# pku-lab-1806-llm/lab-1806-vec-db

Measured on AMD Instinct MI355X. Metric: queries/sec at recall@10, Gist1M d=960 (Flat brute force, L2Sqr, k=10), higher is better.
Workload: dtype f32 (int8 lower-bound filter pass); 1 GPU; flat_knn_gist1m; rows=1000000, dim=960, k=10, dist=L2Sqr, parallelism=single GPU, steps_in_flight=1, queries_per_corpus_pass=128

## Files before the change

lab_1806_vec_db_amd/csrc/api.hip:

```cpp
#include <algorithm>
#include <cmath>
#include <cstring>

#include "ctx.hpp"
#include "pq_hnsw.hpp"

using namespace vdb;

static thread_local std::string g_last_error;
void vdb::set_last_error(const std::string &m) { g_last_error = m; }
void vdb::require_gpu() {
    int cnt = 0;
    hipError_t e = hipGetDeviceCount(&cnt);
    if (e != hipSuccess || cnt <= 0)
        throw Error(VDB_ERR_NOGPU, std::string("no usable HIP device (libvdbhip has no CPU fallback): ") +
                                       hipGetErrorString(e));
}

void vdb::merge_topk_dev(Index &ix, const void *d_dists, const void *d_ids, const void *d_counts, uint64_t stride_d,
                           uint64_t stride_i, uint64_t stride_c, uint64_t n_shards, uint64_t nq, uint64_t k,
                           void *d_out_idx, void *d_out_dist, void *d_out_count, void *stream) {
    VDB_REQUIRE(d_dists && d_ids && d_counts && d_out_idx && d_out_dist && d_out_count, "null argument");
    VDB_REQUIRE(k >= 1 && k <= 1024, "k must be in 1..1024");
    VDB_REQUIRE(nq <= 65535 && n_shards <= 65535, "too many queries or shards for one call");
// ... 414 lines not shown
    idx->ix.flat_mode = mode;
    VDB_API_END
}
int vdb_set_param(vdb_index *idx, const char *name, int64_t value) {
    VDB_API_BEGIN
    VDB_REQUIRE(idx && name, "null argument");
    std::string n(name);
    if (n == "mfma_variant")
        mfma_set_variant((int)value);
    else if (n == "flat_share")
        mfma_set_share((int)value);
    else if (n == "flat_gemm")
        idx->ix.flat_gemm_mode = (int)value;
    else if (n == "hnsw_dma")
        hnsw_set_dma((int)value);
    else if (n == "hnsw_half")
        hnsw_set_half((int)value);
    else if (n == "ivf_half")
        ivf_set_half((int)value);
    else if (n == "ivf_q8")
        ivf_set_q8((int)value);
    else if (n == "hnsw_build_gpu")
        hnsw_set_build_gpu((int)value);
    else if (n == "hnsw_pool_cap")
        hnsw_set_pool_cap((int)value);
    else if (n == "pq_adc_fast")
        pq_set_adc_fast((int)value);
    else if (n == "pq_sample16")
        pq_set_adc16_sample((int)value);
    else if (n == "pq_adc16")
        pq_set_adc16((int)value);
    else if (n == "pq_adc8_sliced")
        pq_set_adc8_sliced((int)value);
    else if (n == "flat_sample_thin")
        mfma_set_sample_thin((int)value);
    else if (n == "flat_gemm_tw")
        gemm_set_tw((int)value);
    else if (n == "flat_gemm_nt")
        gemm_set_nt((int)value);
    else if (n == "flat_gemm_zigzag")
        gemm_set_zigzag((int)value);
    else if (n == "flat_gemm_block_rows") {
        VDB_REQUIRE(value >= 0, "flat_gemm_block_rows must be >= 0");
        gemm_set_block_rows((uint64_t)value);
    }
    else if (n == "flat_gemm_stagger")
        gemm_set_stagger((int)value);
    else if (n == "flat_gemm_debug")
        idx->ix.flat_gemm_debug = (int)value;
    else if (n == "flat_tail")
        idx->ix.flat_tail_mode = (int)value;
    else if (n == "flat_tail_lb_nw")
        flat_tail_lb_set_nw((int)value);
    else if (n == "flat_small")
        idx->ix.flat_small_mode = (int)value;
    else if (n == "flat_small_max_rows")
        idx->ix.flat_small_max_rows = (uint64_t)value;
    else if (n == "flat_half")
        idx->ix.flat_half_mode = (int)value;
    else if (n == "flat_i8")
        idx->ix.flat_i8_mode = (int)value;
    else if (n == "flat_i8_rows") {
        VDB_REQUIRE(value >= 64 && value <= 8192 && value % 64 == 0, "flat_i8_rows must be a multiple of 64 in [64, 8192]");
        idx->ix.flat_i8_kprime = (uint32_t)value;
    }
    else if (n == "debug_alloc_fail_over")
        devbuf_fail_over() = (size_t)value;
    else if (n == "flat_i8_unit_min")
        idx->ix.flat_i8_unit_min = (int)value;
    else if (n == "flat_i8_full")
        idx->ix.flat_i8_full = (int)value;
    else if (n == "flat_i8_refine") {
        idx->ix.flat_i8_refine = (int)value;
        idx->ix.i8_refine_on = 0;
        idx->ix.i8_refine_calls = 0;
    }
    else if (n == "flat_i8_second")
        idx->ix.flat_i8_second = (int)value;
    else if (n == "flat_i8_stats") {
        idx->ix.flat_i8_stats = (int)value;
        for (auto &h : idx->ix.i8_rounds_hist) h = 0;
        idx->ix.i8_hits_sum = 0;
        idx->ix.i8_hits_max = 0;
        idx->ix.i8_stat_queries = 0;
    }
    else if (n == "flat_i8_hits") {
        VDB_REQUIRE(value >= 256 && value <= 4096, "flat_i8_hits must be in [256, 4096]");
        idx->ix.flat_i8_hits = (uint32_t)value;
    }
    else if (n == "flat_gemm8_sample_res")
        gemm8_set_sample_res((int)value);
    else if (n == "flat_gemm8_nt")
        gemm8_set_nt((int)value);
    else if (n == "flat_gemm8_kc")
        gemm8_set_kc((int)value);
    else if (n == "flat_gemm8_burst")
        gemm8_set_burst((int)value);
    else if (n == "flat_gemm8_res")
        gemm8_set_res((int)value);
    else if (n == "flat_gemm8_coop")
        gemm8_set_coop((int)value);
    else if (n == "flat_gemm8_grid")
        gemm8_set_grid((int)value);
    else if (n == "flat_gemm_coop")
        gemm_set_coop((int)value);
    else if (n == "flat_half_kmul") {
        VDB_REQUIRE(value >= 1 && value <= 64, "flat_half_kmul must be in [1, 64]");
        idx->ix.flat_half_kmul = (uint32_t)value;
    }
    else
        throw Error(VDB_ERR_INVALID, "unknown parameter " + n);
    VDB_API_END
}
int vdb_index_prepare(vdb_index *idx, int all_tiers) {
    VDB_API_BEGIN
    VDB_REQUIRE(idx, "null index");
    require_gpu();
    idx->ix.prepare_flat(all_tiers != 0);
    VDB_API_END
}
int vdb_flat_fallback_count(const vdb_index *idx, uint64_t *out) {
    VDB_API_BEGIN
    VDB_REQUIRE(idx && out, "null argument");
    *out = idx->ix.fallback_count.load();
    VDB_API_END
}

int vdb_get_stat(const vdb_index *idx, const char *name, uint64_t *out) {
    VDB_API_BEGIN
    VDB_REQUIRE(idx && name && out, "null argument");
    std::string n(name);
    if (n == "flat_fallback")
        *out = idx->ix.fallback_count.load();
    else if (n == "flat_half_queries")
        *out = idx->ix.half_queries.load();
    else if (n == "flat_half_redo")
        *out = idx->ix.half_redo.load();
    else if (n == "flat_half_valid")
        *out = idx->ix.half_valid ? 1 : 0;
    else if (n == "flat_gemm_coop_sets")
        *out = gemm_last_coop();
    else if (n == "flat_gemm8_coop_sets")
        *out = gemm8_last_coop();
    else if (n == "flat_i8_queries")
        *out = idx->ix.i8_queries.load();
    else if (n == "flat_i8_redo")
        *out = idx->ix.i8_redo.load();
    else if (n == "flat_i8_valid")
        *out = idx->ix.i8_valid.load() ? 1 : 0;
    else if (n.rfind("flat_i8_rounds_", 0) == 0 && n.size() == 16 && n[15] >= '0' && n[15] <= '8')
        *out = idx->ix.i8_rounds_hist[n[15] - '0'].load();
    else if (n == "mirror_alloc_failures")
        *out = idx->ix.mirror_alloc_failures.load();
    else if (n == "flat_i8_second_queries")
        *out = idx->ix.i8_second_queries.load();
    else if (n == "flat_i8_second_redo")
        *out = idx->ix.i8_second_redo.load();
    else if (n == "flat_i8_hits_sum")
        *out = idx->ix.i8_hits_sum.load();
    else if (n == "flat_i8_hits_max")
        *out = idx->ix.i8_hits_max.load();
    else if (n == "flat_i8_stat_queries")
        *out = idx->ix.i8_stat_queries.load();
    else if (n == "flat_i8_rows_walked")
        *out = idx->ix.i8_rows_walked.load();
    else if (n == "flat_bf16_mirror")
        *out = idx->ix.tiled_built ? 1 : 0;
    else if (n == "hnsw_heap_walk_queries")
        *out = idx->ix.hnsw.heap_walk_queries.load();
    else if (n == "hnsw_half_dropped")
        *out = idx->ix.hnsw.last_half_dropped.load();
    else if (n == "ivf_last_offers")
        *out = idx->ix.ivf.last_offers.load();
    else if (n == "ivf_last_rows_fetched_q8")
        *out = idx->ix.ivf.last_rows_fetched_q8.load();
    else if (n == "ivf_last_kept_q8")
        *out = idx->ix.ivf.last_kept_q8.load();
    else if (n == "ivf_last_kept")
        *out = idx->ix.ivf.last_kept.load();
    else if (n == "pq_adc16_queries")
        *out = idx->ix.pq.adc16_queries.load();
    else if (n == "flat_i8_refine_queries")
        *out = idx->ix.i8_refine_queries.load();
    else if (n == "flat_i8_refine_on")
        *out = (uint64_t)idx->ix.i8_refine_on.load();
    else if (n == "pq_q8_overflow")
        *out = idx->ix.pq.q8_overflow.load();
    else if (n == "pq_q8_short")
        *out = idx->ix.pq.q8_short.load();
    else if (n == "pq_q8_hits_sum")
        *out = idx->ix.pq.q8_hits_sum.load();
    else if (n == "pq_q8_hits_max")
        *out = idx->ix.pq.q8_hits_max.load();
    else if (n == "hbm_bytes_per_row")
        *out = idx->ix.hbm_bytes_per_row();
    else
        throw Error(VDB_ERR_INVALID, "unknown statistic " + n);
    VDB_API_END
}

int vdb_pq_attach(vdb_index *idx, uint64_t n_bits, uint64_t m, const float *centroids, const uint8_t *codes) {
    VDB_API_BEGIN
    VDB_REQUIRE(idx && centroids, "null argument");
    pq_attach(idx->ix, n_bits, m, centroids, codes);
    VDB_API_END
}
int vdb_pq_build(vdb_index *idx, uint64_t n_bits, uint64_t m, uint64_t train_n, uint64_t max_iter, float tol,
                 uint64_t seed) {
    VDB_API_BEGIN
    VDB_REQUIRE(idx, "null index");
    pq_build(idx->ix, n_bits, m, train_n, max_iter, tol, seed);
    VDB_API_END
}
int vdb_pq_clear(vdb_index *idx) {
    VDB_API_BEGIN
    VDB_REQUIRE(idx, "null index");
    pq_clear(idx->ix);
    VDB_API_END
}
int vdb_pq_has(const vdb_index *idx, int *out) {
    VDB_API_BEGIN
    VDB_REQUIRE(idx && out, "null argument");
    *out = idx->ix.pq.present ? 1 : 0;
    VDB_API_END
}
int vdb_pq_info(const vdb_index *idx, uint64_t *n_bits, uint64_t *m, uint64_t *enc_dim) {
    VDB_API_BEGIN
    VDB_REQUIRE(idx, "null index");
    VDB_REQUIRE(idx->ix.pq.present, "no PQ table");
    if (n_bits) *n_bits = idx->ix.pq.n_bits;
    if (m) *m = idx->ix.pq.m;
    if (enc_dim) *enc_dim = idx->ix.pq.enc_dim;
    VDB_API_END
}
int vdb_pq_export(const vdb_index *idx, float *centroids, uint8_t *codes) {
    VDB_API_BEGIN
    VDB_REQUIRE(idx, "null index");
    const Index &ix = idx->ix;
    VDB_REQUIRE(ix.pq.present, "no PQ table");
    if (centroids) std::memcpy(centroids, ix.pq.h_centroids.data(), ix.pq.h_centroids.size() * sizeof(float));
    if (codes && ix.n) {
        ix.use_device();
        VDB_HIP(hipMemcpy(codes, ix.pq.d_codes.p, ix.n * ix.pq.enc_dim, hipMemcpyDeviceToHost));
    }
// ... 460 lines not shown
```

lab_1806_vec_db_amd/csrc/index.hip:

```cpp
#include "index.hpp"

#include <algorithm>
#include <cmath>
#include <cstring>

namespace vdb {

Index::Index(int dev, uint64_t d, int ds, bool u8) : device(dev), dim(d), dist(ds), elem_u8(u8) {
#ifndef VDB_HOST_SANITIZER_BUILD
    use_device();
    hipDeviceProp_t prop;
    VDB_HIP(hipGetDeviceProperties(&prop, dev));
    num_cu = prop.multiProcessorCount > 0 ? prop.multiProcessorCount : 256;
    std::string arch = prop.gcnArchName;
    if (arch.rfind("gfx950", 0) != 0)
        throw Error(4, "libvdbhip is built for gfx950 (MI355X) only; device reports " + arch);
#endif
}

std::unique_ptr<Workspace> Index::acquire_ws() {
    use_device();
    {
        std::lock_guard<std::mutex> g(ws_mu);
        if (!ws_free.empty()) {
// ... 626 lines not shown
                                     ws.dense.as<float>(), ld_s, num_cu, s, unit_min ? 1 : 0);
        else if (gemm)
            launch_flat_gemm_sample(xt, n, (uint32_t)dim, ws.qfrag_g.as<float>(), d_qmul, (uint32_t)ngroups,
                                    d_sq.as<float>(), cosine, s_step, ws.dense.as<float>(), ld_s, num_cu, s);
        else
            launch_flat_mfma_sample(d_tiled.as<float>(), n, (uint32_t)dim, ws.qfrag.as<float>(), (uint32_t)nbatch,
                                    d_sq.as<float>(), cosine, s_step, ws.dense.as<float>(), ld_s, num_cu, s);
        if (n_s <= select_tau_max_n()) {
            launch_select_tau(ws.dense.as<float>(), ld_s, (uint32_t)n_s, (uint32_t)nq_pad, (uint32_t)nq, s_rank, d_tau, s);
        } else {
            const uint32_t cap_s = topk_capacity(s_rank);
            launch_topk_dense(ws.dense.as<float>(), ld_s, n_s, (uint32_t)nq_pad, s_rank, ws.lists.as<uint64_t>(), s);
            launch_topk_merge(ws.lists.as<uint64_t>(), nl_s, cap_s, (uint32_t)nq_pad, s_rank, ws.keys_a.as<uint64_t>(), s);
            launch_extract_tau(ws.keys_a.as<uint64_t>(), cap_s, (uint32_t)nq_pad, s_rank, d_tau, s);
        }
        if (nq_pad > nq && n_s > select_tau_max_n())
            VDB_HIP(hipMemsetD32Async(reinterpret_cast<hipDeviceptr_t>(d_tau + nq), (int)0xFF800000u, nq_pad - nq, s));
    }
    uint64_t *d_cand = ws.lists.as<uint64_t>();
    uint32_t *d_sync = d_hits + nq_pad;
    if (!half && !i8) VDB_HIP(hipMemsetAsync(d_hits, 0, (nq_pad + sync_words) * sizeof(uint32_t), s));
    const uint64_t hbm_passes = gemm ? ngroups : (nbatch + mfma_share() - 1) / mfma_share();
    {
        std::lock_guard<std::mutex> g(pass_mu);
        if (pass_ev_valid) VDB_HIP(hipStreamWaitEvent(s, pass_ev, 0));
    }
    prof_begin(ws, i8 ? "flat_i8" : (half ? "flat_half" : "flat_mfma"),
               double(hbm_passes) * double(n) * dim * (i8 ? 1 : (half ? sizeof(uint16_t) : sizeof(float))));
    if (i8)
        launch_flat_gemm8_filter(d_tiled_i8.p, n, (uint32_t)dim, ws.qfrag_g.p, d_qscale, (uint32_t)ngroups, d_rowc_i8.as<float>(), d_tau,
                                 d_cand, d_hits, CAND_CAP, flat_gemm_debug, num_cu, s,
                                 i8_second ? CAND_CAP : std::max<uint32_t>(64u, s_step * s_rank));
    else if (gemm)
        launch_flat_gemm_filter(xt, n, (uint32_t)dim, ws.qfrag_g.as<float>(), d_qmul, (uint32_t)ngroups,
                                d_sq.as<float>(), cosine, d_tau, d_cand, d_hits, CAND_CAP, flat_gemm_debug, num_cu, s);
    else
        launch_flat_mfma_filter(d_tiled.as<float>(), n, (uint32_t)dim, ws.qfrag.as<float>(), (uint32_t)nbatch,
                                d_sq.as<float>(), cosine, d_tau, d_cand, d_hits, CAND_CAP, d_sync, num_cu, s);
    prof_end(ws);
    {
        std::lock_guard<std::mutex> g(pass_mu);
        if (!pass_ev) VDB_HIP(hipEventCreateWithFlags(&pass_ev, hipEventDisableTiming));
        VDB_HIP(hipEventRecord(pass_ev, s));
        pass_ev_valid = true;
    }
    SplitErr se;
    if (half) {
        se.qerr = d_qerr;
        se.dx_abs = half_dx_abs;
        se.dx_rel = half_dx_rel;
    }
    if (i8) {
        se.qoff = d_qoff;
        se.mu_norm = i8_mu_norm;
    }
    if (i8 || (flat_tail_mode != 1 && !elem_u8 && flat_tail64_supported((uint32_t)dim, kprime, ksel))) {
        FlatTailArgs t{};
        t.cand = d_cand;
        t.cap = CAND_CAP;
        t.cnt = d_hits;
        t.kprime = kprime;
        t.ksel = ksel;
        t.kstride = (uint32_t)k;
        t.X = d_rows.as<float>();
        t.dim = (uint32_t)dim;
        t.Q = d_q;
        t.metric = cosine ? MET_COSINE : MET_L2_DIRECT;
        t.xsq = d_sq.as<float>();
        t.qsq = ws.qsq.as<float>();
        t.n_rows = n;
        t.xsq_max = xsq_max;
        t.xsq_min_pos = xsq_min_pos;
        t.cosine = cosine;
        t.se = se;
        t.id_offset = id_offset;
        bool refine = false;
        if (i8 && !i8_second && nq >= 64 && flat_i8_refine != 1) {
            bool on = flat_i8_refine == 2;
            if (flat_i8_refine == 0 && i8_refine_on.load() != 0) on = (i8_refine_calls.fetch_add(1) % 32u) != 31u;
            refine = on && ensure_rows_h(ws);
        }
        const size_t st_off = (nq + 15) & ~size_t(15);
        const bool want_stats = i8 && flat_i8_stats;
        t.flags = static_cast<uint8_t *>(ws.pinned(want_stats ? st_off + nq * sizeof(uint32_t) : nq));
        if (want_stats) t.qstat = reinterpret_cast<uint32_t *>(t.flags + st_off);
        p.stats = want_stats;
        p.refined = refine;
        if (refine) {
            launch_flat_refine_half(d_rows_h.as<uint16_t>(), (uint32_t)dim, half_sx(), half_dx_abs, half_dx_rel, cosine, d_q, d_sq.as<float>(),
                                    ws.qsq.as<float>(), d_qoff, d_cand, CAND_CAP, d_hits, (uint32_t)nq, CAND_CAP, s);
            i8_refine_queries += nq;
        }
        t.out_idx = d_idx;
        t.out_dist = d_dist;
        t.out_count = d_cnt;
        t.tau = d_tau;
        if (i8 && i8_second && nq <= 96 && flat_i8_full != 1) {
            ws.keys_b.reserve(nq * size_t(CAND_CAP) * sizeof(uint64_t));
            launch_flat_full_lb(t, (uint32_t)nq, ws.keys_b.as<uint64_t>(), ws.keys_c.as<uint64_t>(), s);
        } else if (i8)
            launch_flat_tail_lb(t, (uint32_t)nq, s);
        else
            launch_flat_tail64(t, (uint32_t)nq, s);
    } else {
        launch_topk_merge_counted(d_cand, CAND_CAP, d_hits, (uint32_t)nq, kprime, ws.keys_a.as<uint64_t>(), s);
        rerank_rows((uint32_t)dim, d_q, (uint32_t)nq, cosine ? MET_COSINE : MET_L2_DIRECT, d_sq.as<float>(),
                      ws.qsq.as<float>(), ws.keys_a.as<uint64_t>(), ws.keys_b.as<uint64_t>(), kprime, capp, s);
        launch_topk_merge(ws.keys_b.as<uint64_t>(), 1, capp, (uint32_t)nq, ksel, ws.keys_c.as<uint64_t>(), s);
        launch_flat_finish(ws.keys_c.as<uint64_t>(), capk, ws.keys_a.as<uint64_t>(), capp, (uint32_t)nq, ksel, (uint32_t)k, kprime,
                           n, ws.qsq.as<float>(), xsq_max, xsq_min_pos, cosine, (uint32_t)dim, se, d_hits, CAND_CAP, id_offset,
                           static_cast<uint8_t *>(ws.pinned(nq)), d_idx, d_dist, d_cnt, s);
    }
    p.active = true;
    p.half = half;
    p.i8 = i8;
    p.i8_second = i8_second;
    p.kprime = kprime;
    p.ksel = ksel;
    p.nq = nq;
    p.k = k;
    p.d_q = d_q;
    p.d_idx = d_idx;
    p.d_dist = d_dist;
    p.d_cnt = d_cnt;
}

void Index::flat_knn_finish(Workspace &ws, FlatPending &p) {
    hipStream_t s = ws.stream;
    if (!p.active) return;
    p.active = false;
    const bool half = p.half, i8 = p.i8, i8_second = p.i8_second;
    const uint32_t kprime = p.kprime, ksel = p.ksel;
    const uint64_t nq = p.nq, k = p.k;
    const float *d_q = p.d_q;
    uint64_t *d_idx = p.d_idx;
    float *d_dist = p.d_dist;
    uint64_t *d_cnt = p.d_cnt;
    const uint8_t *flags = static_cast<const uint8_t *>(ws.pinned(nq));
    VDB_SYNC(s);
    std::vector<uint64_t> redo;
    for (uint64_t q = 0; q < nq; q++)
        if (flags[q] & 1u) redo.push_back(q);
    if (half) {
        half_queries += nq;
        half_redo += redo.size();
    }
    if (i8 && i8_second) {
        i8_second_queries += nq;
        i8_second_redo += redo.size();
    }
    const bool try_second = i8 && !i8_second && flat_i8_second != 1 && !redo.empty();
    if (i8 && !i8_second) {
        i8_queries += nq;
        if (!try_second) i8_redo += redo.size();
        if (flat_i8_refine == 0 && nq >= 64) {
            uint64_t rs = 0;
            for (uint64_t q = 0; q < nq; q++) rs += std::min<uint32_t>(flags[q] >> 1, 32u);
            const double mean_rounds = double(rs) / double(nq);
            if (!p.refined) {
                const int was = i8_refine_on.load();
                const int now = was ? (mean_rounds >= 4.0 ? 1 : 0) : (mean_rounds >= 6.0 ? 1 : 0);
                if (now != was) {
                    i8_refine_on = now;
                    i8_refine_calls = 0;
                }
            }
        }
        if (flat_i8_stats) {
            const uint32_t *qs = reinterpret_cast<const uint32_t *>(flags + ((nq + 15) & ~size_t(15)));
            uint64_t hs = 0, hm = 0;
            for (uint64_t q = 0; q < nq; q++) {
                const uint32_t r = qs[q] & 0xFFu, h = qs[q] >> 8;
                i8_rounds_hist[r < 8 ? r : 8] += 1;
                hs += h;
                hm = std::max<uint64_t>(hm, h);
            }
            i8_hits_sum += hs;
            i8_stat_queries += nq;
            uint64_t cur = i8_hits_max.load();
            while (hm > cur && !i8_hits_max.compare_exchange_weak(cur, hm)) {
            }
        }
    }
    if (redo.empty()) return;
    if (!half && !i8) fallback_count += redo.size();
    const uint64_t nr = redo.size();
    DevBuf rx, rq, rqs, ri, rd, rc, rdk;
    rx.reserve(nr * sizeof(uint64_t));
    rq.reserve(nr * dim * sizeof(float));
    rqs.reserve(nr * sizeof(float));
    ri.reserve(nr * k * sizeof(uint64_t));
    rd.reserve(nr * k * sizeof(float));
    rc.reserve(nr * sizeof(uint64_t));
    VDB_HIP(hipMemcpyAsync(rx.p, redo.data(), nr * sizeof(uint64_t), hipMemcpyHostToDevice, s));
    launch_gather_rows_f32(d_q, rx.as<uint64_t>(), nr, (uint32_t)dim, rq.as<float>(), s);
    launch_gather_rows_f32(ws.qsq.as<float>(), rx.as<uint64_t>(), nr, 1, rqs.as<float>(), s);
    if (try_second) {
        rdk.reserve(nr * sizeof(float));
        launch_gather_dk(d_dist, d_cnt, rx.as<uint64_t>(), nr, (uint32_t)k, ksel, rdk.as<float>(), s);
    }
    VDB_HIP(hipMemsetAsync(ri.p, 0, nr * k * sizeof(uint64_t), s));
    VDB_HIP(hipMemsetAsync(rd.p, 0, nr * k * sizeof(float), s));
    VDB_SYNC(s);
    if (try_second) {
        const uint64_t before = i8_second_redo.load();
        flat_knn_device(ws, rq.as<float>(), nr, k, ri.as<uint64_t>(), rd.as<float>(), rc.as<uint64_t>(), true, 0, true, rdk.as<float>());
        i8_redo += i8_second_redo.load() - before;
    } else if (i8)
        flat_knn_device(ws, rq.as<float>(), nr, k, ri.as<uint64_t>(), rd.as<float>(), rc.as<uint64_t>(), true, 0, false);
    else if (half)
        flat_knn_device(ws, rq.as<float>(), nr, k, ri.as<uint64_t>(), rd.as<float>(), rc.as<uint64_t>(), false, kprime);
    else
        flat_exact_device(ws, rq.as<float>(), rqs.as<float>(), nr, ksel, k, ri.as<uint64_t>(), rd.as<float>(), rc.as<uint64_t>());
    launch_scatter_results(ri.as<uint64_t>(), rd.as<float>(), rc.as<uint64_t>(), rx.as<uint64_t>(), nr, (uint32_t)k, d_idx, d_dist, d_cnt, s);
    VDB_SYNC(s);
}

void Index::flat_debug_keys(Workspace &ws, const float *d_q, uint64_t nq, int tier, float *h_keys, float *h_qsq, float *h_qerr,
                            float *h_dx) {
    hipStream_t s = ws.stream;
    VDB_REQUIRE(nq >= 1 && nq <= 1024 && n >= 1, "debug keys: 1..1024 queries on a non-empty index");
    VDB_REQUIRE(mfma_supported((uint32_t)dim), "debug keys: the dimension has no MFMA shortlist path");
    const int cosine = dist == 1 ? 1 : 0;
    const uint64_t gq = gemm_group(), ngroups = (nq + gq - 1) / gq, nq_pad = ngroups * gq;
    if (tier == 2) {
        VDB_REQUIRE(!elem_u8 && (dim & 3) == 0 && gemm8_supported((uint32_t)dim), "debug keys: the index has no 8-bit pass");
        VDB_REQUIRE(ensure_i8(ws), "debug keys: the 8-bit mirror could not be allocated");
        const uint64_t n_s8 = gemm8_sample_rows(n, 1), ld8 = (n_s8 + 63) & ~63ull;
        ws.qsq.reserve(nq_pad * sizeof(float));
        ws.qfrag_g.reserve(nq_pad * size_t(mfma_dim_pad((uint32_t)dim)));
        ws.dense.reserve(nq_pad * ld8 * sizeof(float));
        ws.qaux.reserve(2 * nq_pad * sizeof(float));
        ws.misc.reserve((nq_pad + 128) * sizeof(uint32_t));
        float *d_qs8 = ws.qaux.as<float>(), *d_qoff = d_qs8 + nq_pad;
        launch_query_prep_i8(d_q, (uint32_t)nq, (uint32_t)nq_pad, (uint32_t)dim, d_mu_i8.as<float>(), i8_l1, i8_l2, ws.qsq.as<float>(), d_qs8,
                             d_qoff, ws.misc.as<uint32_t>(), ws.qfrag_g.p, s, cosine);
        launch_flat_gemm8_sample(d_tiled_i8.p, n, (uint32_t)dim, ws.qfrag_g.p, d_qs8, (uint32_t)ngroups, d_rowc_i8.as<float>(), 1,
                                 ws.dense.as<float>(), ld8, num_cu, s);
        VDB_HIP(hipMemcpy2DAsync(h_keys, n * sizeof(float), ws.dense.p, ld8 * sizeof(float), n * sizeof(float), nq, hipMemcpyDeviceToHost, s));
        if (h_qsq) VDB_HIP(hipMemcpyAsync(h_qsq, ws.qsq.p, nq * sizeof(float), hipMemcpyDeviceToHost, s));
        if (h_qerr) VDB_HIP(hipMemcpyAsync(h_qerr, d_qoff, nq * sizeof(float), hipMemcpyDeviceToHost, s));
        VDB_SYNC(s);
        if (h_dx) {
            h_dx[0] = i8_l1;
            h_dx[1] = i8_l2;
            h_dx[2] = i8_mu_norm;
            h_dx[3] = 0.0f;
        }
        return;
    }
    const bool half = tier == 0;
    VDB_REQUIRE(!half || ensure_half(ws), "debug keys: the index holds no fp16 mirror");
    if (!half) VDB_REQUIRE(ensure_tiled(ws), "debug keys: the split-bf16 mirror could not be allocated");
    const uint64_t n_s = gemm_sample_rows(n, 1), ld = (n_s + 63) & ~63ull;
    ws.qsq.reserve(nq_pad * sizeof(float));
    ws.qfrag_g.reserve(nq_pad * size_t(mfma_dim_pad((uint32_t)dim)) * sizeof(float));
    ws.dense.reserve(nq_pad * ld * sizeof(float));
    ws.qaux.reserve(3 * nq_pad * sizeof(float));
// ... 31 lines not shown
```

lab_1806_vec_db_amd/csrc/index.hpp:

```cpp
#pragma once
#include <algorithm>
#include <atomic>
#include <cmath>
#include <cstdlib>
#include <map>
#include <memory>
#include <mutex>
#include <string>
#include <vector>

#include "common.hpp"
#include "kernels.hpp"

namespace vdb {

inline bool devbuf_efence() {
    static const bool on = [] {
        const char *e = std::getenv("VDB_EFENCE");
        return e && e[0] == '1';
    }();
    return on;
}
inline std::atomic<size_t> &devbuf_fail_over() {
    static std::atomic<size_t> v{0};
// ... 65 lines not shown
    double bytes = 0;
};

struct Workspace {
    hipStream_t stream = nullptr;
    DevBuf q, qsq, qfrag, qfrag_g, qaux, dense, lists, keys_a, keys_b, keys_c, flags, out_idx, out_dist, out_cnt, lut, misc;
    DevBuf pq_img16, pq_aux16;
    DevBuf small_part, small_cnt;
    std::vector<std::pair<hipEvent_t, hipEvent_t>> ev_pool;
    struct Pending {
        std::string name;
        size_t ev;
        double bytes;
    };
    std::vector<Pending> pending;
    size_t ev_used = 0;
    void *h_pinned = nullptr;
    size_t h_pinned_cap = 0;
    hipEvent_t order_ev = nullptr;
    void *pinned(size_t bytes) {
        if (bytes > h_pinned_cap) {
            if (h_pinned) (void)hipHostFree(h_pinned);
            h_pinned = nullptr;
            size_t want = bytes < (64u << 10) ? (64u << 10) : bytes;
            VDB_HIP(hipHostMalloc(&h_pinned, want, hipHostMallocDefault));
            h_pinned_cap = want;
        }
        return h_pinned;
    }
    Workspace() {
#ifndef VDB_HOST_SANITIZER_BUILD
        VDB_HIP(hipStreamCreateWithFlags(&stream, hipStreamNonBlocking));
#endif
    }
    ~Workspace() {
        if (h_pinned) (void)hipHostFree(h_pinned);
        if (order_ev) (void)hipEventDestroy(order_ev);
        for (auto &e : ev_pool) {
            (void)hipEventDestroy(e.first);
            (void)hipEventDestroy(e.second);
        }
        if (stream) (void)hipStreamDestroy(stream);
    }
};

struct PQState {
    bool present = false;
    uint64_t n_bits = 0, m = 0, kc = 0, enc_dim = 0;
    uint64_t n_coded = 0;
    std::vector<uint64_t> gstart;
    std::vector<float> h_centroids;
    std::vector<float> h_cent_cache;
    DevBuf d_centroids, d_cent_cache, d_codes, d_gstart;
    DevBuf d_codes_t;
    bool codes_t_valid = false;
    std::atomic<uint64_t> adc16_queries{0};
    std::atomic<uint64_t> q8_overflow{0}, q8_short{0};
    std::atomic<uint64_t> q8_hits_sum{0}, q8_hits_max{0};
};

struct HNSWState {
    bool present = false;
    uint64_t m = 0, max_m0 = 0, ef_construction = 0, default_ef = 0;
    float inv_log_m = 0;
    std::vector<uint32_t> level0;
    std::vector<uint64_t> len0, vec_level, upper_off, upper_len;
    std::vector<uint32_t> upper;
    bool has_enter = false;
    uint64_t enter_point = 0, enter_level = 0;
    uint64_t rng_state = 0;
    bool dev_dirty = true;
    DevBuf d_level0, d_len0, d_upper, d_upper_len, d_upper_off;
    std::atomic<uint64_t> last_n_dist{0}, last_n_expanded{0};
    std::atomic<uint64_t> last_half_dropped{0};
    std::atomic<uint64_t> heap_walk_queries{0};
};

struct FlatPending {
    bool active = false;
    bool half = false;
    bool i8 = false;
    bool i8_second = false;
    bool stats = false;
    bool refined = false;
    uint32_t kprime = 0, ksel = 0;
    uint64_t nq = 0, k = 0;
    const float *d_q = nullptr;
    uint64_t *d_idx = nullptr;
    float *d_dist = nullptr;
    uint64_t *d_cnt = nullptr;
};

struct Index;
struct IVFState {
    bool present = false;
    uint64_t k = 0, default_n_probes = 4;
    std::shared_ptr<Index> cent;
    std::vector<uint64_t> assign;
    std::vector<uint32_t> offsets;
    std::vector<uint32_t> sizes_desc;
    DevBuf d_offsets, d_members;
    std::atomic<uint64_t> last_rows_fetched_q8{0};
    std::atomic<uint64_t> last_kept_q8{0};
    std::atomic<uint32_t> q8_overflows{0};
    std::atomic<uint64_t> last_offers{0}, last_kept{0};
    std::atomic<uint32_t> half_overflows{0};
};

struct Index {
    int device = 0;
    int num_cu = 256;
    uint64_t dim = 0;
    int dist = 0;
    uint64_t n = 0;
    uint64_t id_offset = 0;
    bool elem_u8 = false;
    size_t elem_size() const { return elem_u8 ? 1 : sizeof(float); }
    const float *rows_f32_view(DevBuf &scratch, uint64_t r0, uint64_t r1, hipStream_t s) const;
    template <class F>
    void for_tile_chunks(Workspace &ws, uint64_t t_begin, uint64_t t_end, uint64_t n_rows, F fn) const {
        if (!elem_u8) {
            fn(d_rows.as<float>(), t_begin, t_end, std::min(t_begin * 16, n_rows), n_rows);
            return;
        }
        constexpr uint64_t CH = 12 * 64;
        ws.dense.reserve(CH * 16 * dim * sizeof(float));
        for (uint64_t t = t_begin; t < t_end; t += CH) {
            const uint64_t tb = std::min(t_end, t + CH), ra = std::min(t * 16, n_rows), rb = std::min(tb * 16, n_rows);
            fn(rows_f32_view(ws.dense, ra, rb, ws.stream), t, tb, ra, rb);
        }
    }
    DevBuf d_rows, d_sq;
    DevBuf d_tiled;
    std::atomic<bool> tiled_built{false};
    std::mutex tiled_mu;
    bool ensure_tiled(Workspace &ws);
    uint64_t tiled_failed_n = ~0ull, half_failed_n = ~0ull, i8_failed_n = ~0ull;
    std::atomic<uint64_t> mirror_alloc_failures{0};
    void prepare_flat(bool all_tiers);
    uint64_t hbm_bytes_per_row() const;
    DevBuf d_tiled_h, d_half_err;
    bool half_valid = false;
    int half_exp = 0;
    float half_dx_abs = 0.0f, half_dx_rel = 0.0f;
    int flat_half_mode = 0;
    uint32_t flat_half_kmul = 4;
    std::atomic<uint64_t> half_queries{0}, half_redo{0};
    void half_refresh(Workspace &ws, uint64_t n_old, uint64_t n_new);
    uint64_t half_n = 0;
    std::mutex half_mu;
    bool i8_defers_half() const;
    bool ensure_half(Workspace &ws);
    float half_sx() const { return std::ldexp(1.0f, 13 - half_exp); }
    DevBuf d_tiled_i8, d_rowc_i8, d_mu_i8;
    std::atomic<bool> i8_valid{false};
    uint64_t i8_n = 0;
    uint64_t i8_mu_rows = 0;
    float i8_l1 = 0.0f, i8_l2 = 0.0f, i8_mu_norm = 0.0f;
    int flat_i8_mode = 0;
    uint32_t flat_i8_kprime = 2048;
    int flat_i8_full = 0;
    int flat_i8_refine = 0;
    std::atomic<int> i8_refine_on{0};
    std::atomic<uint32_t> i8_refine_calls{0};
    std::atomic<uint64_t> i8_refine_queries{0};
    int flat_i8_unit_min = 0;
    int flat_i8_second = 0;
    std::atomic<uint64_t> i8_second_queries{0}, i8_second_redo{0};
    uint32_t flat_i8_hits = 1024;
    std::atomic<uint64_t> i8_queries{0}, i8_redo{0};
    int flat_i8_stats = 0;
    std::atomic<uint64_t> i8_rounds_hist[9] = {};
    std::atomic<uint64_t> i8_hits_sum{0}, i8_hits_max{0}, i8_stat_queries{0};
    std::atomic<uint64_t> i8_rows_walked{0};
    std::mutex i8_mu;
    bool i8_applicable(uint32_t ksel) const;
    bool ensure_i8(Workspace &ws);
    void ensure_i8_locked(Workspace &ws);
    DevBuf d_rows_h;
    uint64_t rows_h_n = 0;
    uint64_t rows_h_failed_n = ~0ull;
    int rows_h_exp = 0;
    std::mutex rows_h_mu;
    bool ensure_rows_h(Workspace &ws);
    DevBuf d_rows_q8, d_q8_scale, d_q8_err;
    uint64_t rows_q8_n = 0;
    std::mutex rows_q8_mu;
    bool ensure_rows_q8(Workspace &ws);
    std::vector<float> h_sq;
    float xsq_max = 0.0f;
    float xsq_min_pos = 3.4e38f;
    mutable std::vector<float> h_rows;
    mutable bool host_valid = true;
    mutable std::mutex host_mu;
    int flat_mode = 0;
    int flat_gemm_mode = 0;
    int flat_gemm_debug = 0;
    int flat_tail_mode = 0;
    int flat_small_mode = 0;
    uint64_t flat_small_max_rows = 16384;
    bool flat_small_applies(uint64_t nq, uint64_t k) const;
    void flat_small_device(Workspace &ws, const float *q, uint64_t nq, uint64_t k, uint64_t *o_idx, float *o_dist, uint64_t *o_cnt);
    std::atomic<uint64_t> fallback_count{0};
    PQState pq;
    HNSWState hnsw;
    IVFState ivf;

    std::mutex ws_mu;
    std::vector<std::unique_ptr<Workspace>> ws_free;
    std::mutex pass_mu;
    hipEvent_t pass_ev = nullptr;
    bool pass_ev_valid = false;
    bool prof_on = false;
    std::mutex prof_mu;
    std::map<std::string, ProfEntry> prof;

    Index(int dev, uint64_t d, int ds, bool u8 = false);
    ~Index() {
        if (pass_ev) (void)hipEventDestroy(pass_ev);
    }
    void use_device() const {
#ifndef VDB_HOST_SANITIZER_BUILD
        VDB_HIP(hipSetDevice(device));
#endif
    }
    std::unique_ptr<Workspace> acquire_ws();
    void release_ws(std::unique_ptr<Workspace> ws);
    const float *host_rows() const;

    void add_rows(const void *rows, uint64_t count, bool on_device);
    void swap_remove(uint64_t i);

    void prof_begin(Workspace &ws, const char *name, double bytes);
    void prof_end(Workspace &ws);
    void prof_collect(Workspace &ws);

    void flat_knn_device(Workspace &ws, const float *d_q, uint64_t nq, uint64_t k, uint64_t *d_idx, float *d_dist,
                         uint64_t *d_cnt, bool allow_half = true, uint32_t kprime_min = 0, bool allow_i8 = true,
                         const float *d_dk_hint = nullptr);
    void flat_knn_enqueue(Workspace &ws, const float *d_q, uint64_t nq, uint64_t k, uint64_t *d_idx, float *d_dist, uint64_t *d_cnt,
                          bool allow_half, uint32_t kprime_min, FlatPending &p, bool allow_i8 = true, const float *d_dk_hint = nullptr);
    void flat_knn_finish(Workspace &ws, FlatPending &p);
    void flat_sorted_device(Workspace &ws, const float *d_q, uint64_t nq, uint64_t ksel, uint64_t k, uint64_t *d_idx,
                            float *d_dist, uint64_t *d_cnt);
    void scan_rows(uint64_t nrows, uint32_t d, const float *Q, uint32_t nq, int metric, const float *xsq, const float *qsq, float *out,
                   uint64_t ld, bool use_lds, hipStream_t s) const;
    void rerank_rows(uint32_t d, const float *Q, uint32_t nq, int metric, const float *xsq, const float *qsq, const uint64_t *cand,
                     uint64_t *out, uint32_t ncand, uint32_t ldc, hipStream_t s) const;
    void flat_debug_keys(Workspace &ws, const float *d_q, uint64_t nq, int tier, float *h_keys, float *h_qsq, float *h_qerr,
                         float *h_dx );
    void flat_exact_device(Workspace &ws, const float *d_q, const float *d_qsq, uint64_t nq, uint32_t ksel,
                           uint64_t k, uint64_t *d_idx, float *d_dist, uint64_t *d_cnt);
};

struct WsLease {
    Index &ix;
// ... 9 lines not shown
```

lab_1806_vec_db_amd/csrc/k_exact.hip:

```cpp
#include <algorithm>
#include <atomic>
#include <cstdio>
#include <cstdlib>
#include <vector>

#include "common.hpp"
#include "kernels.hpp"

#pragma clang fp contract(off)

namespace vdb {

enum Fold : int { FOLD_L2 = 0, FOLD_DOT = 1 };

template <int FOLD>
__device__ __forceinline__ float fold1(float acc, float x, float q) {
    if (FOLD == FOLD_L2) {
        float df = x - q;
        float sq = df * df;
        return acc + sq;
    } else {
        float p = x * q;
        return acc + p;
    }
// ... 735 lines not shown
                sorted = sort64(skeys[lane], lane);
                const uint64_t ek = __shfl(sorted, kk - 1), ak = sbest[0][a.kprime - 1];
                uint8_t f = 1;
                if (lane == 0)
                    f = flat_certify_flag(ek, ak, q, a.kprime, a.n_rows, a.qsq, a.xsq_max, a.xsq_min_pos, a.cosine, a.dim, a.se, cnt_q, a.cap);
                flag = (uint8_t)__shfl((int)f, 0);
            }
        }
    }
    if (wave != 0) return;
    const bool ok = lane < a.ksel && sorted != PAIR_NONE;
    if (lane < a.ksel) {
        a.out_idx[uint64_t(q) * a.kstride + lane] = ok ? uint64_t(uint32_t(sorted)) + a.id_offset : 0;
        a.out_dist[uint64_t(q) * a.kstride + lane] = ok ? f32_from_orderable(uint32_t(sorted >> 32)) : 0.0f;
    }
    const uint32_t count = __builtin_popcountll(__ballot(ok));
    if (lane == 0) {
        if (a.out_count) a.out_count[q] = count;
        a.flags[q] = flag;
    }
}
bool flat_tail64_supported(uint32_t dim, uint32_t kprime, uint32_t ksel) {
    return (dim & 3) == 0 && dim >= 64 && dim <= 8192 && kprime >= 1 && kprime <= 64 && ksel >= 1 && ksel <= 64;
}
void launch_flat_tail64(const FlatTailArgs &a, uint32_t nq, hipStream_t s) {
    if (nq == 0) return;
    VDB_REQUIRE(flat_tail64_supported(a.dim, a.kprime, a.ksel), "flat_tail64: unsupported shape");
    const size_t lds = (size_t(a.dim / 4) + 4 * 72) * sizeof(float4);
    if (a.metric == MET_L2_DIRECT)
        hipLaunchKernelGGL((k_flat_tail64<FOLD_L2>), dim3(nq), dim3(256), lds, s, a);
    else
        hipLaunchKernelGGL((k_flat_tail64<FOLD_DOT>), dim3(nq), dim3(256), lds, s, a);
    VDB_HIP(hipGetLastError());
}

#define TAIL_LB_AUTO_NW(nq) 40
template <int NW>
__device__ __forceinline__ uint64_t block_top64_above(const uint64_t *__restrict__ src, uint32_t total, uint64_t (*sbest)[64], uint64_t above) {
    const uint32_t lane = threadIdx.x & 63, wave = threadIdx.x >> 6;
    const uint32_t batches = (total + 255) / 256;
    uint64_t best = PAIR_NONE;
    for (uint32_t bt = wave; bt < batches; bt += NW) {
        uint64_t r[4];
#pragma unroll
        for (int u = 0; u < 4; u++) {
            const uint32_t i = (bt * 4 + u) * 64 + lane;
            const uint64_t v = i < total ? src[i] : PAIR_NONE;
            r[u] = v > above ? v : PAIR_NONE;
        }
        const uint64_t tau = __shfl(best, 63);
        uint64_t lo = r[0] < r[1] ? r[0] : r[1], lo2 = r[2] < r[3] ? r[2] : r[3];
        lo = lo < lo2 ? lo : lo2;
        if (__ballot(lo < tau) == 0) continue;
        bitonic_sort_from<2, 4>(r, lane);
        const uint64_t a = merge64(r[0], r[1], lane), b = merge64(r[2], r[3], lane);
        best = merge64(best, merge64(a, b, lane), lane);
    }
    sbest[wave][lane] = best;
    __syncthreads();
    if (wave != 0) return PAIR_NONE;
    uint64_t m = sbest[0][lane];
#pragma unroll
    for (int w = 1; w < NW; w++) m = merge64(m, sbest[w][lane], lane);
    return m;
}
__device__ __forceinline__ uint8_t flat_certify_lb(uint64_t ek, float kappa, uint32_t q, const FlatTailArgs &a) {
    if (ek == PAIR_NONE) return 1;
    const float dk = f32_from_orderable(uint32_t(ek >> 32));
    if (a.cosine) {
        const float qs = a.qsq[q], qn = sqrtf(qs);
        const bool plain = a.xsq_min_pos >= 1e-30f && qs >= 1e-30f && qs <= 1e30f && sqrtf(a.xsq_min_pos) * qn > 1e-9f;
        const float nr = 2.0f + 2.0f * a.se.mu_norm;
        float lower = 0.5f * (kappa + a.se.qoff[q]);
        lower = lower - 4.0f * 5.9604645e-8f * fabsf(lower) - float(2 * a.dim + 16) * 5.9604645e-8f * 1.01f - 2.0f * 5.9604645e-8f * nr * nr;
        return (plain && dk < lower) ? 0 : 1;
    }
    const float qn = sqrtf(a.qsq[q]);
    const float rx = fminf(sqrtf(a.xsq_max), (qn + sqrtf(fmaxf(dk, 0.0f))) * 1.001f);
    const float nr = rx + qn + 2.0f * a.se.mu_norm;
    float lower = kappa + a.se.qoff[q];
    lower = lower - float(a.dim + 8) * 5.9604645e-8f * 1.01f * fabsf(lower) - 4.0f * 5.9604645e-8f * nr * nr;
    return dk < lower ? 0 : 1;
}
template <int FOLD, int NW, int PCD>
__global__ __launch_bounds__(NW * 64, PCD ? 4 : 1) void k_flat_tail_lb(FlatTailArgs a) {
    constexpr bool PC = PCD != 0;
    static_assert(NW == 8 || NW == 4 || NW == 2 || NW == 1, "a stage covers the 64 keys of a round");
    static_assert(!PC || NW == 4, "producer / consumer fold: four waves");
    constexpr int RW = 64 / NW, NP = RW / 8;
    constexpr int DEPTH = PC ? PCD : (NW == 8 ? 8 : (NW == 4 ? 4 : (NW == 2 ? 3 : 2)));
    extern __shared__ float4 ftl_smem[];
    __shared__ uint64_t sbest[NW][64];
    __shared__ uint64_t skeys[64];
    __shared__ uint32_t s_flag;
    const uint32_t q = blockIdx.x, lane = threadIdx.x & 63, wave = threadIdx.x >> 6;
    const uint32_t d4 = a.dim / 4;
    float4 *qs4 = ftl_smem, *tile = ftl_smem + d4 + wave * (RW * 9);
    for (uint32_t i = threadIdx.x; i < d4; i += NW * 64) qs4[i] = reinterpret_cast<const float4 *>(a.Q + uint64_t(q) * a.dim)[i];
    const uint32_t cnt_q = a.cnt[q];
    const uint32_t total = cnt_q <= a.cap ? cnt_q : 0;
    const uint32_t kk = a.ksel;
    const float tau_q = a.tau[q];
    uint64_t run = PAIR_NONE;
    uint64_t above = 0;
    uint8_t flag = 1;
    const uint32_t rounds = cnt_q <= a.cap ? a.kprime / 64 : 0;
#ifdef VDB_TAIL_STAMPS
    uint32_t ns = 0;
#define TAIL_STAMP()                                                                                      \
    do {                                                                                                  \
        if (a.stamps && threadIdx.x == 0 && ns < 30) a.stamps[q * 32 + ns++] = __builtin_readcyclecounter(); \
    } while (0)
#else
#define TAIL_STAMP() do { } while (0)
#endif
    TAIL_STAMP();
    uint32_t rounds_done = 0;
    for (uint32_t rd = 0; rd < rounds; rd++) {
        rounds_done = rd + 1;
        const uint64_t best = block_top64_above<NW>(a.cand + uint64_t(q) * a.cap, total, sbest, above);
        __syncthreads();
        if (wave == 0) sbest[0][lane] = best;
        if (threadIdx.x < 64) skeys[threadIdx.x] = PAIR_NONE;
        __syncthreads();
        TAIL_STAMP();
        uint32_t idx[NP];
        bool live[NP];
#pragma unroll
        for (int i = 0; i < NP; i++) {
            const uint32_t j = wave * RW + 8 * i + (lane >> 3);
            const uint64_t c = sbest[0][j];
            live[i] = c != PAIR_NONE && j < 63;
            idx[i] = live[i] ? uint32_t(c) : 0u;
#if defined(VDB_TAIL_ABLATE) && VDB_TAIL_ABLATE == 1
            idx[i] &= 63u;
#endif
        }
        float acc;
        if constexpr (PC) {
            const bool consumer = wave == (blockIdx.x & 3u);
            acc = pc_rerank_fold<FOLD, DEPTH>(a.X, a.dim, idx, live, qs4, ftl_smem + d4, wave, lane, consumer);
            const uint64_t c = sbest[0][lane];
            if (consumer && c != PAIR_NONE && lane < 63)
                skeys[lane] = pair_key(FOLD == FOLD_L2 ? acc : epilogue(MET_COSINE, acc, a.xsq[uint32_t(c)], a.qsq[q]), uint32_t(c));
        } else {
            if constexpr (NW == 8)
                acc = group_rerank_fold<FOLD, 8>(a.X, a.dim, idx[0], live[0], qs4, tile, lane);
            else
                acc = group_rerank_fold_n<FOLD, DEPTH, RW>(a.X, a.dim, idx, live, qs4, tile, lane);
            const uint32_t j = wave * RW + lane / NW;
            const uint64_t c = sbest[0][j];
            if (c != PAIR_NONE && j < 63 && lane % NW == 0)
                skeys[j] = pair_key(FOLD == FOLD_L2 ? acc : epilogue(MET_COSINE, acc, a.xsq[uint32_t(c)], a.qsq[q]), uint32_t(c));
        }
        __syncthreads();
        TAIL_STAMP();
        if (wave == 0) {
            run = merge64(run, sort64(skeys[lane], lane), lane);
            const uint64_t ek = __shfl(run, kk - 1), nxt = sbest[0][63];
            if (lane == 0) {
                const float kappa = nxt == PAIR_NONE ? tau_q : f32_from_orderable(uint32_t(nxt >> 32));
                s_flag = flat_certify_lb(ek, kappa, q, a) | (nxt == PAIR_NONE ? 2u : 0u);
            }
        }
        __syncthreads();
        TAIL_STAMP();
        const uint32_t f = s_flag;
        if ((f & 1u) == 0) {
            flag = 0;
            break;
        }
        if (f & 2u) break;
        above = sbest[0][62];
        __syncthreads();
    }
#ifdef VDB_TAIL_STAMPS
    if (a.stamps && threadIdx.x == 0) {
        a.stamps[q * 32 + 30] = ns;
        a.stamps[q * 32 + 31] = total;
    }
#endif
    if (wave != 0) return;
    const bool ok = lane < a.ksel && run != PAIR_NONE;
    if (lane < a.ksel) {
        a.out_idx[uint64_t(q) * a.kstride + lane] = ok ? uint64_t(uint32_t(run)) + a.id_offset : 0;
        a.out_dist[uint64_t(q) * a.kstride + lane] = ok ? f32_from_orderable(uint32_t(run >> 32)) : 0.0f;
    }
    const uint32_t count = __builtin_popcountll(__ballot(ok));
    if (lane == 0) {
        if (a.out_count) a.out_count[q] = count;
        a.flags[q] = uint8_t(flag | ((rounds_done < 127u ? rounds_done : 127u) << 1));
        if (a.qstat) a.qstat[q] = rounds_done | ((cnt_q < 0xFFFFFFu ? cnt_q : 0xFFFFFFu) << 8);
    }
}
bool flat_tail_lb_supported(uint32_t dim, uint32_t kprime, uint32_t ksel) {
    return (dim & 3) == 0 && dim >= 64 && dim <= 8192 && kprime >= 64 && kprime % 64 == 0 && kprime <= 8192 && ksel >= 1 && ksel <= 64;
}
static std::atomic<int> g_tail_lb_nw{0};
void flat_tail_lb_set_nw(int v) { g_tail_lb_nw = v; }
#ifdef VDB_TAIL_STAMPS
static void tail_stamps_report(unsigned long long *d, uint32_t nq, hipStream_t s) {
    VDB_SYNC(s);
    std::vector<unsigned long long> h(size_t(nq) * 32);
    VDB_HIP(hipMemcpy(h.data(), d, h.size() * 8, hipMemcpyDeviceToHost));
    VDB_HIP(hipFree(d));
    uint32_t hist[8] = {0}, nr = 0;
    double sel = 0, fold = 0, cert = 0, life = 0;
    for (uint32_t q = 0; q < nq; q++) {
        const unsigned long long *t = &h[size_t(q) * 32];
        const uint32_t ns = (uint32_t)t[30], r = ns ? (ns - 1) / 3 : 0;
        hist[r < 7 ? r : 7]++;
        if (ns) life += double(t[ns - 1] - t[0]);
        for (uint32_t i = 0; i < r; i++, nr++) {
            sel += double(t[1 + 3 * i] - t[3 * i]);
            fold += double(t[2 + 3 * i] - t[1 + 3 * i]);
            cert += double(t[3 + 3 * i] - t[2 + 3 * i]);
        }
    }
    fprintf(stderr, "TAIL_STAMPS nq %u  queries by rounds 0:%u 1:%u 2:%u 3:%u 4:%u 5+:%u  ticks per round: select %.0f fold %.0f merge+certify %.0f  per workgroup %.0f\n",
            nq, hist[0], hist[1], hist[2], hist[3], hist[4], hist[5] + hist[6] + hist[7], sel / (nr ? nr : 1), fold / (nr ? nr : 1),
            cert / (nr ? nr : 1), life / nq);
}
#endif
void launch_flat_tail_lb(const FlatTailArgs &a0, uint32_t nq, hipStream_t s) {
    if (nq == 0) return;
    FlatTailArgs a = a0;
#ifdef VDB_TAIL_STAMPS
    static std::atomic<int> calls{0};
    const char *want = getenv("VDB_TAIL_STAMPS");
    unsigned long long *stamps = nullptr;
    if (want && ++calls == atoi(want)) {
        VDB_HIP(hipMalloc(&stamps, size_t(nq) * 32 * 8));
        VDB_HIP(hipMemset(stamps, 0, size_t(nq) * 32 * 8));
        a.stamps = stamps;
    }
#endif
    VDB_REQUIRE(flat_tail_lb_supported(a.dim, a.kprime, a.ksel) && (a.metric == MET_L2_DIRECT || a.metric == MET_COSINE) && a.se.qoff && a.tau,
                "flat_tail_lb: unsupported shape");
    VDB_REQUIRE((a.metric == MET_COSINE) == (a.cosine != 0) && (a.metric == MET_L2_DIRECT || (a.xsq && a.qsq)), "flat_tail_lb: metric / norms");
    const size_t lds = (size_t(a.dim / 4) + 2 * 64 * 9) * sizeof(float4);
    int nw = g_tail_lb_nw;
    if (nw != 8 && nw != 4 && nw != 2 && nw != 1 && nw != 40 && nw != 41) nw = TAIL_LB_AUTO_NW(nq);
    if (a.metric == MET_COSINE) {
        if (nw == 8)
            hipLaunchKernelGGL((k_flat_tail_lb<FOLD_DOT, 8, 0>), dim3(nq), dim3(512), lds, s, a);
        else if (nw == 41)
            hipLaunchKernelGGL((k_flat_tail_lb<FOLD_DOT, 4, 5>), dim3(nq), dim3(256), lds, s, a);
        else
            hipLaunchKernelGGL((k_flat_tail_lb<FOLD_DOT, 4, 3>), dim3(nq), dim3(256), lds, s, a);
    } else if (nw == 40)
        hipLaunchKernelGGL((k_flat_tail_lb<FOLD_L2, 4, 3>), dim3(nq), dim3(256), lds, s, a);
    else if (nw == 41)
        hipLaunchKernelGGL((k_flat_tail_lb<FOLD_L2, 4, 5>), dim3(nq), dim3(256), lds, s, a);
    else if (nw == 8)
        hipLaunchKernelGGL((k_flat_tail_lb<FOLD_L2, 8, 0>), dim3(nq), dim3(512), lds, s, a);
    else if (nw == 4)
        hipLaunchKernelGGL((k_flat_tail_lb<FOLD_L2, 4, 0>), dim3(nq), dim3(256), lds, s, a);
    else if (nw == 2)
        hipLaunchKernelGGL((k_flat_tail_lb<FOLD_L2, 2, 0>), dim3(nq), dim3(128), lds, s, a);
    else
        hipLaunchKernelGGL((k_flat_tail_lb<FOLD_L2, 1, 0>), dim3(nq), dim3(64), lds, s, a);
    VDB_HIP(hipGetLastError());
#ifdef VDB_TAIL_STAMPS
    if (stamps) tail_stamps_report(stamps, nq, s);
#endif
}

__global__ __launch_bounds__(64) void k_flat_finish_lb(FlatTailArgs a, const uint64_t *__restrict__ exact_sorted, uint32_t lde) {
    const uint32_t q = blockIdx.x, lane = threadIdx.x;
    const uint32_t cnt_q = a.cnt[q];
    const uint64_t e = lane < a.ksel ? exact_sorted[uint64_t(q) * lde + lane] : PAIR_NONE;
    const uint64_t ek = __shfl(e, a.ksel - 1);
    uint8_t flag = 1;
    if (lane == 0 && cnt_q <= a.cap) flag = flat_certify_lb(ek, a.tau[q], q, a);
    const bool ok = lane < a.ksel && e != PAIR_NONE;
    if (lane < a.ksel) {
        a.out_idx[uint64_t(q) * a.kstride + lane] = ok ? uint64_t(uint32_t(e)) + a.id_offset : 0;
        a.out_dist[uint64_t(q) * a.kstride + lane] = ok ? f32_from_orderable(uint32_t(e >> 32)) : 0.0f;
    }
    const uint32_t count = __builtin_popcountll(__ballot(ok));
    if (lane == 0) {
        if (a.out_count) a.out_count[q] = count;
        a.flags[q] = flag;
        if (a.qstat) a.qstat[q] = 0xFFu | ((cnt_q < 0xFFFFFFu ? cnt_q : 0xFFFFFFu) << 8);
    }
}
void launch_flat_full_lb(const FlatTailArgs &a, uint32_t nq, uint64_t *exact_keys , uint64_t *topk ,
                         hipStream_t s) {
    if (nq == 0) return;
    VDB_REQUIRE(a.ksel >= 1 && a.ksel <= 64 && (a.dim & 3) == 0 && a.se.qoff && a.tau, "flat_full_lb: unsupported shape");
    launch_rerank(a.X, a.dim, a.Q, nq, a.metric, a.xsq, a.qsq, a.cand, exact_keys, a.cap, a.cap, s, a.cnt);
    launch_topk_merge_counted(exact_keys, a.cap, a.cnt, nq, a.ksel, topk, s);
    hipLaunchKernelGGL(k_flat_finish_lb, dim3(nq), dim3(64), 0, s, a, topk, topk_capacity(a.ksel));
    VDB_HIP(hipGetLastError());
}

void launch_certify(const uint64_t *exact_sorted, uint32_t lde, const uint64_t *approx_sorted, uint32_t lda,
                    uint32_t nq, uint32_t k, uint32_t kprime, uint64_t n_rows, const float *qsq, float xsq_max,
                    float xsq_min_pos, int cosine, uint32_t dim, uint8_t *flags, hipStream_t s) {
    if (nq == 0) return;
    hipLaunchKernelGGL(k_certify, dim3((nq + 63) / 64), dim3(64), 0, s, exact_sorted, lde, approx_sorted, lda, nq, k,
                       kprime, n_rows, qsq, xsq_max, xsq_min_pos, cosine, dim, flags);
}

}
```

Measured before the change: 1.056 million queries/s.

## Build a sorted survivor hit-list after first tail round to avoid rescanning candidates

After the first rerank round in the int8 lower-bound tail kernel, one extra pass over the candidate list keeps only candidates that the current k-th exact distance cannot certify away. Up to 256 survivors are rank-sorted in shared memory. Later rounds take 63-entry slices from this list plus a sentinel for the smallest excluded key, instead of rerunning the block-wide top-64 selection over the whole candidate buffer. The change adds shared memory (about 4KB) and an O(m^2) sort, which may lower occupancy, and it also records a passes statistic.

```diff
diff --git a/lab_1806_vec_db_amd/csrc/api.hip b/lab_1806_vec_db_amd/csrc/api.hip
--- a/lab_1806_vec_db_amd/csrc/api.hip
+++ b/lab_1806_vec_db_amd/csrc/api.hip
@@ -520,6 +520,7 @@
         for (auto &h : idx->ix.i8_rounds_hist) h = 0;
         idx->ix.i8_hits_sum = 0;
         idx->ix.i8_hits_max = 0;
+        idx->ix.i8_passes_max = 0;
         idx->ix.i8_stat_queries = 0;
     }
     else if (n == "flat_i8_hits") {
@@ -598,6 +599,8 @@
         *out = idx->ix.i8_hits_sum.load();
     else if (n == "flat_i8_hits_max")
         *out = idx->ix.i8_hits_max.load();
+    else if (n == "flat_i8_hitlist_passes_max")
+        *out = idx->ix.i8_passes_max.load();
     else if (n == "flat_i8_stat_queries")
         *out = idx->ix.i8_stat_queries.load();
     else if (n == "flat_i8_rows_walked")
diff --git a/lab_1806_vec_db_amd/csrc/index.hip b/lab_1806_vec_db_amd/csrc/index.hip
--- a/lab_1806_vec_db_amd/csrc/index.hip
+++ b/lab_1806_vec_db_amd/csrc/index.hip
@@ -732,9 +732,10 @@
         }
         const size_t st_off = (nq + 15) & ~size_t(15);
         const bool want_stats = i8 && flat_i8_stats;
-        t.flags = static_cast<uint8_t *>(ws.pinned(want_stats ? st_off + nq * sizeof(uint32_t) : nq));
+        t.flags = static_cast<uint8_t *>(ws.pinned(want_stats ? st_off + 2 * nq * sizeof(uint32_t) : nq));
         if (want_stats) t.qstat = reinterpret_cast<uint32_t *>(t.flags + st_off);
         p.stats = want_stats;
+        p.stats_off = st_off;
         p.refined = refine;
         if (refine) {
             launch_flat_refine_half(d_rows_h.as<uint16_t>(), (uint32_t)dim, half_sx(), half_dx_abs, half_dx_rel, cosine, d_q, d_sq.as<float>(),
@@ -816,14 +817,18 @@
                 }
             }
         }
-        if (flat_i8_stats) {
-            const uint32_t *qs = reinterpret_cast<const uint32_t *>(flags + ((nq + 15) & ~size_t(15)));
-            uint64_t hs = 0, hm = 0;
+        if (p.stats) {
+            const uint32_t *qs = reinterpret_cast<const uint32_t *>(flags + p.stats_off);
+            uint64_t hs = 0, hm = 0, pm = 0;
             for (uint64_t q = 0; q < nq; q++) {
                 const uint32_t r = qs[q] & 0xFFu, h = qs[q] >> 8;
                 i8_rounds_hist[r < 8 ? r : 8] += 1;
                 hs += h;
                 hm = std::max<uint64_t>(hm, h);
+                pm = std::max<uint64_t>(pm, qs[nq + q]);
+            }
+            uint64_t pc = i8_passes_max.load();
+            while (pm > pc && !i8_passes_max.compare_exchange_weak(pc, pm)) {
             }
             i8_hits_sum += hs;
             i8_stat_queries += nq;
diff --git a/lab_1806_vec_db_amd/csrc/index.hpp b/lab_1806_vec_db_amd/csrc/index.hpp
--- a/lab_1806_vec_db_amd/csrc/index.hpp
+++ b/lab_1806_vec_db_amd/csrc/index.hpp
@@ -171,6 +171,7 @@
     bool i8 = false;
     bool i8_second = false;
     bool stats = false;
+    size_t stats_off = 0;
     bool refined = false;
     uint32_t kprime = 0, ksel = 0;
     uint64_t nq = 0, k = 0;
@@ -261,6 +262,7 @@
     int flat_i8_stats = 0;
     std::atomic<uint64_t> i8_rounds_hist[9] = {};
     std::atomic<uint64_t> i8_hits_sum{0}, i8_hits_max{0}, i8_stat_queries{0};
+    std::atomic<uint64_t> i8_passes_max{0};
     std::atomic<uint64_t> i8_rows_walked{0};
     std::mutex i8_mu;
     bool i8_applicable(uint32_t ksel) const;
diff --git a/lab_1806_vec_db_amd/csrc/k_exact.hip b/lab_1806_vec_db_amd/csrc/k_exact.hip
--- a/lab_1806_vec_db_amd/csrc/k_exact.hip
+++ b/lab_1806_vec_db_amd/csrc/k_exact.hip
@@ -841,6 +841,7 @@
     lower = lower - float(a.dim + 8) * 5.9604645e-8f * 1.01f * fabsf(lower) - 4.0f * 5.9604645e-8f * nr * nr;
     return dk < lower ? 0 : 1;
 }
+#define TAIL_LB_R2 256u
 template <int FOLD, int NW, int PCD>
 __global__ __launch_bounds__(NW * 64, PCD ? 4 : 1) void k_flat_tail_lb(FlatTailArgs a) {
     constexpr bool PC = PCD != 0;
@@ -852,9 +853,17 @@
     __shared__ uint64_t sbest[NW][64];
     __shared__ uint64_t skeys[64];
     __shared__ uint32_t s_flag;
+    __shared__ uint64_t s_ek;
+    __shared__ uint64_t s2_raw[TAIL_LB_R2], s2[TAIL_LB_R2];
+    __shared__ uint32_t s2_n;
+    __shared__ unsigned long long s2_excl;
     const uint32_t q = blockIdx.x, lane = threadIdx.x & 63, wave = threadIdx.x >> 6;
     const uint32_t d4 = a.dim / 4;
     float4 *qs4 = ftl_smem, *tile = ftl_smem + d4 + wave * (RW * 9);
+    if (threadIdx.x == 0) {
+        s2_n = 0;
+        s2_excl = PAIR_NONE;
+    }
     for (uint32_t i = threadIdx.x; i < d4; i += NW * 64) qs4[i] = reinterpret_cast<const float4 *>(a.Q + uint64_t(q) * a.dim)[i];
     const uint32_t cnt_q = a.cnt[q];
     const uint32_t total = cnt_q <= a.cap ? cnt_q : 0;
@@ -874,13 +883,29 @@
 #define TAIL_STAMP() do { } while (0)
 #endif
     TAIL_STAMP();
-    uint32_t rounds_done = 0;
+    uint32_t rounds_done = 0, passes = 0;
+    bool s2_tried = false;
+    uint32_t s2_len = 0, s2_pos = 0;
+    uint64_t s2_min_excl = PAIR_NONE;
     for (uint32_t rd = 0; rd < rounds; rd++) {
+        if (s2_len) {
+            if (s2_pos >= s2_len) break;
+            if (threadIdx.x < 64) {
+                const uint32_t p = s2_pos + threadIdx.x;
+                uint64_t v = p < s2_len ? s2[p] : PAIR_NONE;
+                if (threadIdx.x == 63) v = v < s2_min_excl ? v : s2_min_excl;
+                sbest[0][threadIdx.x] = v;
+                skeys[threadIdx.x] = PAIR_NONE;
+            }
+            s2_pos += 63;
+        } else {
+            const uint64_t best = block_top64_above<NW>(a.cand + uint64_t(q) * a.cap, total, sbest, above);
+            passes++;
+            __syncthreads();
+            if (wave == 0) sbest[0][lane] = best;
+            if (threadIdx.x < 64) skeys[threadIdx.x] = PAIR_NONE;
+        }
         rounds_done = rd + 1;
-        const uint64_t best = block_top64_above<NW>(a.cand + uint64_t(q) * a.cap, total, sbest, above);
-        __syncthreads();
-        if (wave == 0) sbest[0][lane] = best;
-        if (threadIdx.x < 64) skeys[threadIdx.x] = PAIR_NONE;
         __syncthreads();
         TAIL_STAMP();
         uint32_t idx[NP];
@@ -920,6 +945,7 @@
             if (lane == 0) {
                 const float kappa = nxt == PAIR_NONE ? tau_q : f32_from_orderable(uint32_t(nxt >> 32));
                 s_flag = flat_certify_lb(ek, kappa, q, a) | (nxt == PAIR_NONE ? 2u : 0u);
+                s_ek = ek;
             }
         }
         __syncthreads();
@@ -932,6 +958,44 @@
         if (f & 2u) break;
         above = sbest[0][62];
         __syncthreads();
+        if (!s2_tried && rd + 1 < rounds) {
+            s2_tried = true;
+            passes++;
+            const uint64_t ek = s_ek;
+            const uint64_t *src = a.cand + uint64_t(q) * a.cap;
+            uint64_t mn = PAIR_NONE;
+            for (uint32_t i0 = wave * 64; i0 < total; i0 += NW * 64) {
+                const uint32_t i = i0 + lane;
+                const uint64_t v = i < total ? src[i] : PAIR_NONE;
+                bool in = false;
+                if (v != PAIR_NONE && v > above) {
+                    if (flat_certify_lb(ek, f32_from_orderable(uint32_t(v >> 32)), q, a))
+                        in = true;
+                    else
+                        mn = v < mn ? v : mn;
+                }
+                const uint64_t bal = __ballot(in);
+                uint32_t base = 0;
+                if (lane == 0 && bal) base = atomicAdd(&s2_n, (uint32_t)__popcll(bal));
+                base = __shfl(base, 0);
+                const uint32_t slot = base + (uint32_t)__popcll(bal & ((1ull << lane) - 1ull));
+                if (in && slot < TAIL_LB_R2) s2_raw[slot] = v;
+            }
+            if (mn != PAIR_NONE) atomicMin(&s2_excl, (unsigned long long)mn);
+            __syncthreads();
+            const uint32_t m = s2_n;
+            if (m <= TAIL_LB_R2) {
+                for (uint32_t t = threadIdx.x; t < m; t += NW * 64) {
+                    const uint64_t v = s2_raw[t];
+                    uint32_t r = 0;
+                    for (uint32_t j = 0; j < m; j++) r += (s2_raw[j] < v || (s2_raw[j] == v && j < t)) ? 1u : 0u;
+                    s2[r] = v;
+                }
+                s2_len = m;
+                s2_min_excl = s2_excl;
+                __syncthreads();
+            }
+        }
     }
 #ifdef VDB_TAIL_STAMPS
     if (a.stamps && threadIdx.x == 0) {
@@ -949,7 +1013,10 @@
     if (lane == 0) {
         if (a.out_count) a.out_count[q] = count;
         a.flags[q] = uint8_t(flag | ((rounds_done < 127u ? rounds_done : 127u) << 1));
-        if (a.qstat) a.qstat[q] = rounds_done | ((cnt_q < 0xFFFFFFu ? cnt_q : 0xFFFFFFu) << 8);
+        if (a.qstat) {
+            a.qstat[q] = rounds_done | ((cnt_q < 0xFFFFFFu ? cnt_q : 0xFFFFFFu) << 8);
+            a.qstat[gridDim.x + q] = passes;
+        }
     }
 }
 bool flat_tail_lb_supported(uint32_t dim, uint32_t kprime, uint32_t ksel) {
@@ -1041,7 +1108,10 @@
     if (lane == 0) {
         if (a.out_count) a.out_count[q] = count;
         a.flags[q] = flag;
-        if (a.qstat) a.qstat[q] = 0xFFu | ((cnt_q < 0xFFFFFFu ? cnt_q : 0xFFFFFFu) << 8);
+        if (a.qstat) {
+            a.qstat[q] = 0xFFu | ((cnt_q < 0xFFFFFFu ? cnt_q : 0xFFFFFFu) << 8);
+            a.qstat[gridDim.x + q] = 1;
+        }
     }
 }
 void launch_flat_full_lb(const FlatTailArgs &a, uint32_t nq, uint64_t *exact_keys , uint64_t *topk ,
```

Result: no change. 1.064 million queries/s (median of 6 runs) (+0.8%).
